# Tavish9/freegaussian

Measured on AMD Instinct MI355X. Metric: Mpixels/s fwd+bwd @ 1M Gaussians 1080p, higher is better.
Workload: dtype f32; 1 GPU; north-star cfg4: 1000000 Gaussians, 1920x1080, SH degree 3, 1 view per rank per step, view = (rank + step) mod 8 around the 8-view ring, fwd+bwd, RGB, absgrad; layout=uniform, N=1000000, P=2073600, parallelism=view-dp1

## Files before the change

freegaussian_amd/csrc/fg_common.h:

```cpp
#pragma once
#include <hip/hip_runtime.h>
#include <stdint.h>

#include "../../include/fgraster.h"

#define FG_WAVE 64

#define FG_RETURN_IF_LAUNCH_FAILED()                  \
  do {                                                \
    if (hipGetLastError() != hipSuccess) return FG_ERR_LAUNCH; \
  } while (0)

static inline hipStream_t fg_hip_stream(fg_stream_t s) { return reinterpret_cast<hipStream_t>(s); }

#define FG_ALPHA_SKIP (1.0f / 255.0f)
#define FG_ALPHA_MAX 0.999f
#define FG_T_STOP 1e-4f
#define FG_FOV_CLAMP 1.3f

namespace fg {

__device__ __forceinline__ int lane_id() { return __lane_id(); }

__device__ __forceinline__ int alpha_extent(float o, float a, float b, float c, float& ex, float& ey) {
// ... 213 lines not shown
  __builtin_amdgcn_wave_barrier();
  __builtin_amdgcn_fence(__ATOMIC_ACQUIRE, "wavefront");
  float r = 0.f;
  if ((lane >> 2) < ROWS) {
    const float4* src = reinterpret_cast<const float4*>(buf + (lane >> 2) * FG_RED_STRIDE + (lane & 3) * 16);
    const float4 a = src[0], b = src[1], c = src[2], d = src[3];
    r = (((a.x + a.y) + (a.z + a.w)) + ((b.x + b.y) + (b.z + b.w))) +
        (((c.x + c.y) + (c.z + c.w)) + ((d.x + d.y) + (d.z + d.w)));
    r += dpp_mov<FG_DPP_QUAD_XOR1>(r);
    r += dpp_mov<FG_DPP_QUAD_XOR2>(r);
  }
  return r;
}

}
```

freegaussian_amd/csrc/preprocess.hip:

```cpp
#include "project_math.h"
#include "sh_math.h"
#include "slab_io.h"

#include <stdlib.h>

namespace {
using namespace fgp;
using namespace fgsh;

constexpr int REC = FG_SPLAT_FLOATS;
constexpr int RSTRIDE = 20;
constexpr int JAC = FG_SH_JAC_FLOATS;
constexpr int JSTRIDE = 11;

struct FeatLayout {
  int sh_degree;
  int k_stored;
  int n_color;
  int with_depth;
  int n_extra;
};

struct RawForm {
  int enabled;
// ... 267 lines not shown
}

template <bool NOTE>
__global__ void __launch_bounds__(BLOCK) __attribute__((amdgpu_waves_per_eu(NOTE ? FG_PRE_BWD_WAVES : 3)))
preprocess_bwd_kernel(int N, FeatLayout fl, RawForm raw, float* __restrict__ v_d_quats,
                      float* __restrict__ v_d_scales, float* __restrict__ v_features_rest,
                      float* __restrict__ v_rgb, int v_rgb_floats,
                      const float* __restrict__ means, const float* __restrict__ quats,
                      const float* __restrict__ scales, const float* __restrict__ opacities,
                      const float* __restrict__ colors, const float* __restrict__ viewmat,
                      const float* __restrict__ K, int width, int height, float eps2d, int antialiased,
                      const int32_t* __restrict__ radii, const float* __restrict__ v_splats,
                      const float* __restrict__ v_means2d, int m2_stride, const float* __restrict__ v_depths,
                      const float* __restrict__ v_conics, float* __restrict__ v_means, float* __restrict__ v_quats,
                      float* __restrict__ v_scales, float* __restrict__ v_opacities, float* __restrict__ v_colors,
                      float* __restrict__ v_extra, const float* __restrict__ sh_jac, int skip_culled) {
  __shared__ float lds[HROWS * ROW];
  __shared__ uint8_t row_live[BLOCK];
  const int row0 = blockIdx.x * BLOCK;
  const int nrows = min(BLOCK, N - row0);
  const int i = row0 + threadIdx.x;
  const int kk = fl.sh_degree >= 0 ? (fl.sh_degree + 1) * (fl.sh_degree + 1) : 0;
  const bool active = (i < N) && radii[i] > 0;
  float sh_dx = 0.f, sh_dy = 0.f, sh_dz = 1.f, sh_inv = 0.f;
  auto view_direction = [&]() { view_dir(viewmat, means[3 * i], means[3 * i + 1], means[3 * i + 2], sh_dx, sh_dy, sh_dz, sh_inv); };
  if (!NOTE && active && kk > 0) view_direction();
  ShSums sums;
#pragma unroll
  for (int c = 0; c < 3; ++c) sums.col[c] = 0.f;
#pragma unroll
  for (int c = 0; c < 9; ++c) sums.jac[c] = 0.f;
// ... 125 lines not shown
    v_scales[3 * i] = g_s[0]; v_scales[3 * i + 1] = g_s[1]; v_scales[3 * i + 2] = g_s[2];
    v_opacities[i] = g_o;
  }
  if (v_rgb && i < N) {
    float* o = v_rgb + (size_t)v_rgb_floats * i;
    o[0] = vr; o[1] = vg; o[2] = vb;
    if (v_rgb_floats == 6) {
      o[3] = sh_dx; o[4] = sh_dy; o[5] = sh_dz;
    }
  }
  if (kk > 0 && v_colors) {
    float basis[16];
#pragma unroll
    for (int k = 0; k < 16; ++k) basis[k] = 0.f;
    if (active) sh_basis(fl.sh_degree, sh_dx, sh_dy, sh_dz, basis);
#pragma unroll
    for (int h = 0; h < 2; ++h) {
      const int r0 = row0 + h * HROWS, nr = min(HROWS, nrows - h * HROWS);
      if (nr <= 0) break;
      __syncthreads();
      if ((int)(threadIdx.x / HROWS) == h) {
        float* row = lds + (threadIdx.x & (HROWS - 1)) * ROW;
#pragma unroll
        for (int k = 0; k < 16; ++k) {
          const float bk = (k < kk) ? basis[k] : 0.f;
          row[3 * k] = bk * vr; row[3 * k + 1] = bk * vg; row[3 * k + 2] = bk * vb;
        }
      }
      __syncthreads();
      if (raw.enabled) {
        lds_to_slab_at<ROW, true, HROWS>(v_colors + (size_t)r0 * 3, lds, 0, nr, 3, 3);
        if (fl.k_stored > 1)
          lds_to_slab_at<ROW, true, HROWS>(v_features_rest + (size_t)r0 * 3 * (fl.k_stored - 1), lds, 3, nr,
                                           3 * (fl.k_stored - 1), 45);
      } else {
        lds_to_slab_at<ROW, true, HROWS>(v_colors + (size_t)r0 * 3 * fl.k_stored, lds, 0, nr, 3 * fl.k_stored, 48);
      }
    }
  }
}

constexpr int VM_BLOCK = 256, VM_GRID_MAX = 1024, VM_VALUES = 15;
__global__ void __launch_bounds__(VM_BLOCK)
viewmat_bwd_kernel(int N, FeatLayout fl, RawForm raw, const float* __restrict__ means, const float* __restrict__ quats,
                   const float* __restrict__ scales, const float* __restrict__ opacities, const float* __restrict__ colors,
                   const float* __restrict__ viewmat, const float* __restrict__ K, int width, int height, float eps2d,
                   int antialiased, const int32_t* __restrict__ radii, const float* __restrict__ v_splats,
                   const float* __restrict__ v_means2d, int m2_stride, const float* __restrict__ v_depths,
                   const float* __restrict__ v_conics, const float* __restrict__ sh_jac, float* __restrict__ partials) {
  __shared__ float red[VM_BLOCK / 64][16];
  float acc[VM_VALUES];
// ... 169 lines not shown
                     depths, conics, compensations, tiles_touched, splats, depth_keys,
                     reinterpret_cast<int2*>(tile_rects), reinterpret_cast<unsigned long long*>(tile_masks), sh_jac,
                     skip_culled_rows());
  FG_RETURN_IF_LAUNCH_FAILED();
  return FG_OK;
}

int launch_preprocess_bwd(int N, RawForm raw, float* v_d_quats, float* v_d_scales, float* v_features_rest,
                          float* v_rgb, int v_rgb_floats,
                          const float* means, const float* quats, const float* scales, const float* opacities,
                          const float* colors, int sh_degree, int k_stored, int n_color, int with_depth, int n_extra,
                          const float* viewmat, const float* K, int width, int height, float eps2d, int antialiased,
                          const int32_t* radii, const float* v_splats, const float* v_means2d, int v_means2d_stride,
                          const float* v_depths, const float* v_conics, float* v_means, float* v_quats,
                          float* v_scales, float* v_opacities, float* v_colors, float* v_extra,
                          const float* sh_jac, fg_stream_t stream) {
  FeatLayout fl{sh_degree, k_stored, sh_degree >= 0 ? 3 : n_color, with_depth ? 1 : 0, n_extra};
  if (N < 0 || width <= 0 || height <= 0 || !layout_ok(fl) || v_means2d_stride < 2) return FG_ERR_INVALID_ARG;
  if (N == 0) return FG_OK;
  if (!means || !quats || !scales || !opacities || !viewmat || !K || !radii || !v_splats || !v_means2d ||
      !v_means || !v_quats || !v_scales || !v_opacities)
    return FG_ERR_INVALID_ARG;
  if ((fl.n_color > 0 && (!colors || (!v_colors && !(v_rgb && sh_degree >= 0)))) || (n_extra > 0 && !v_extra))
    return FG_ERR_INVALID_ARG;
  if (v_rgb && sh_degree < 0) return FG_ERR_UNSUPPORTED;
  if (v_rgb && v_rgb_floats != 3 && v_rgb_floats != 6) return FG_ERR_INVALID_ARG;
  if (raw.enabled) {
    if (sh_degree < 0 || (k_stored > 1 && (!raw.features_rest || (!v_features_rest && !v_rgb)))) return FG_ERR_INVALID_ARG;
    if (v_rgb && (v_colors || v_features_rest)) return FG_ERR_INVALID_ARG;
    if ((raw.d_quats != nullptr) != (v_d_quats != nullptr) || (raw.d_scales != nullptr) != (v_d_scales != nullptr))
      return FG_ERR_INVALID_ARG;
  }
  const bool note = sh_jac != nullptr && sh_degree >= 1;
  hipLaunchKernelGGL(note ? preprocess_bwd_kernel<true> : preprocess_bwd_kernel<false>, dim3((N + BLOCK - 1) / BLOCK),
                     dim3(BLOCK), 0, fg_hip_stream(stream), N, fl, raw, v_d_quats, v_d_scales, v_features_rest, v_rgb, v_rgb_floats, means, quats, scales, opacities, colors,
                     viewmat, K, width, height, eps2d, antialiased, radii, v_splats, v_means2d, v_means2d_stride,
                     v_depths, v_conics, v_means, v_quats, v_scales, v_opacities, v_colors, v_extra, sh_jac,
                     skip_culled_rows());
  FG_RETURN_IF_LAUNCH_FAILED();
  return FG_OK;
}

}

extern "C" int fg_preprocess_fwd(int N, const float* means, const float* quats, const float* scales,
                                 const float* opacities, const float* colors, int sh_degree, int k_stored,
                                 int n_color, int with_depth, const float* extra, int n_extra,
                                 const float* viewmat, const float* K, int width, int height, float eps2d,
                                 float near_plane, float far_plane, float radius_clip, int tile_size,
                                 int antialiased, int32_t* radii, float* means2d, float* depths, float* conics,
                                 float* compensations, int32_t* tiles_touched, float* splats,
                                 uint32_t* depth_keys, int32_t* tile_rects, uint64_t* tile_masks, float* sh_jac,
                                 fg_stream_t stream) {
  return launch_preprocess_fwd(N, RawForm{0, nullptr, nullptr, nullptr}, means, quats, scales, opacities, colors,
                               sh_degree, k_stored, n_color, with_depth, extra, n_extra, viewmat, K, width, height,
                               eps2d, near_plane, far_plane, radius_clip, tile_size, antialiased, radii, means2d,
                               depths, conics, compensations, tiles_touched, splats, depth_keys, tile_rects, tile_masks,
                               sh_jac, stream);
}

extern "C" int fg_preprocess_bwd(int N, const float* means, const float* quats, const float* scales,
                                 const float* opacities, const float* colors, int sh_degree, int k_stored,
                                 int n_color, int with_depth, int n_extra, const float* viewmat, const float* K,
                                 int width, int height, float eps2d, int antialiased, const int32_t* radii,
                                 const float* v_splats, const float* v_means2d, int v_means2d_stride,
                                 const float* v_depths, const float* v_conics, float* v_means, float* v_quats,
                                 float* v_scales, float* v_opacities, float* v_colors, float* v_extra,
                                 const float* sh_jac, fg_stream_t stream) {
  return launch_preprocess_bwd(N, RawForm{0, nullptr, nullptr, nullptr}, nullptr, nullptr, nullptr, nullptr, 3, means, quats,
                               scales, opacities, colors, sh_degree, k_stored, n_color, with_depth, n_extra, viewmat,
                               K, width, height, eps2d, antialiased, radii, v_splats, v_means2d, v_means2d_stride,
                               v_depths, v_conics, v_means, v_quats, v_scales, v_opacities, v_colors, v_extra,
                               sh_jac, stream);
}

extern "C" int fg_preprocess_raw_fwd(int N, const float* means, const float* quats, const float* d_quats,
                                     const float* log_scales, const float* d_scales,
                                     const float* opacity_logits, const float* features_dc,
                                     const float* features_rest, int sh_degree, int k_stored, int with_depth,
                                     const float* extra, int n_extra, const float* viewmat, const float* K,
                                     int width, int height, float eps2d, float near_plane, float far_plane,
                                     float radius_clip, int tile_size, int antialiased, int32_t* radii,
                                     float* means2d, float* depths, float* conics, float* compensations,
                                     int32_t* tiles_touched, float* splats, uint32_t* depth_keys,
                                     int32_t* tile_rects, uint64_t* tile_masks, float* sh_jac, fg_stream_t stream) {
  return launch_preprocess_fwd(N, RawForm{1, d_quats, d_scales, features_rest}, means, quats, log_scales,
                               opacity_logits, features_dc, sh_degree, k_stored, 3, with_depth, extra, n_extra,
                               viewmat, K, width, height, eps2d, near_plane, far_plane, radius_clip, tile_size,
                               antialiased, radii, means2d, depths, conics, compensations, tiles_touched, splats,
                               depth_keys, tile_rects, tile_masks, sh_jac, stream);
}

extern "C" int fg_preprocess_raw_bwd(int N, const float* means, const float* quats, const float* d_quats,
                                     const float* log_scales, const float* d_scales,
                                     const float* opacity_logits, const float* features_dc,
                                     const float* features_rest, int sh_degree, int k_stored, int with_depth,
                                     int n_extra, const float* viewmat, const float* K, int width, int height,
                                     float eps2d, int antialiased, const int32_t* radii, const float* v_splats,
                                     const float* v_means2d, int v_means2d_stride, const float* v_depths,
                                     const float* v_conics, float* v_means, float* v_quats, float* v_d_quats,
                                     float* v_log_scales, float* v_d_scales, float* v_opacity_logits,
                                     float* v_features_dc, float* v_features_rest, float* v_extra,
                                     const float* sh_jac, fg_stream_t stream) {
  return launch_preprocess_bwd(N, RawForm{1, d_quats, d_scales, features_rest}, v_d_quats, v_d_scales,
                               v_features_rest, nullptr, 3, means, quats, log_scales, opacity_logits, features_dc, sh_degree,
                               k_stored, 3, with_depth, n_extra, viewmat, K, width, height, eps2d, antialiased, radii,
                               v_splats, v_means2d, v_means2d_stride, v_depths, v_conics, v_means, v_quats,
                               v_log_scales, v_opacity_logits, v_features_dc, v_extra, sh_jac, stream);
}

extern "C" int fg_preprocess_raw_bwd_factored(
    int N, const float* means, const float* quats, const float* d_quats, const float* log_scales, const float* d_scales,
    const float* opacity_logits, const float* features_dc, const float* features_rest, int sh_degree, int k_stored,
    int with_depth, int n_extra, const float* viewmat, const float* K, int width, int height, float eps2d, int antialiased,
    const int32_t* radii, const float* v_splats, const float* v_means2d, int v_means2d_stride, const float* v_depths,
    const float* v_conics, float* v_means, float* v_quats, float* v_d_quats, float* v_log_scales, float* v_d_scales,
    float* v_opacity_logits, float* v_rgb, int v_rgb_floats, float* v_extra, const float* sh_jac, fg_stream_t stream) {
  if (!v_rgb) return FG_ERR_INVALID_ARG;
  return launch_preprocess_bwd(N, RawForm{1, d_quats, d_scales, features_rest}, v_d_quats, v_d_scales, nullptr, v_rgb,
                               v_rgb_floats, means, quats, log_scales, opacity_logits, features_dc, sh_degree, k_stored, 3,
                               with_depth, n_extra, viewmat, K, width, height, eps2d, antialiased, radii, v_splats,
                               v_means2d, v_means2d_stride, v_depths, v_conics, v_means, v_quats, v_log_scales,
                               v_opacity_logits, nullptr, v_extra, sh_jac, stream);
// ... 76 lines not shown
```

freegaussian_amd/csrc/raster.hip:

```cpp
#include "fg_common.h"

#include <stdlib.h>
#include <string.h>

#include <type_traits>

#include "jobs_build.h"

namespace {
using namespace fgjobs;

constexpr int TILE = 16;

__host__ __device__ constexpr int rec_vec4(int C) { return (6 + C + 3) / 4; }

__device__ __forceinline__ int tile_of_block(int b, int n, int tile_w, int tile_h, int mode) {
  const int xcd = b & 7, k = b >> 3;
  const int only = ((mode >> 8) & 15) - 1, kmod = mode >> 12;
  mode &= 255;
  if (only >= 0 && xcd != only) return -1;
  if (kmod > 1 && k % kmod != 0) return -1;
  if (mode == 0) {
    const int row = (k / tile_w) * 8 + xcd;
    return row < tile_h ? row * tile_w + (k % tile_w) : -1;
// ... 1412 lines not shown
template <int C, int PPT>
__global__ void __launch_bounds__(256 / PPT)
raster_bwd_kernel(int width, int height, int tile_w, int tile_h, int order_mode, const float4* __restrict__ splats,
                  const int32_t* __restrict__ tile_offsets, const int32_t* __restrict__ flatten_ids,
                  const float* __restrict__ alphas, const int32_t* __restrict__ last_ids,
                  const float* __restrict__ v_render, const float* __restrict__ v_alphas,
                  float* __restrict__ v_splats, Composite comp) {
  constexpr int NW = 256 / PPT / 64;
  __shared__ BwdShared<C, 64 * NW> sh;
  const int tile = tile_of_block(blockIdx.x, tile_w * tile_h, tile_w, tile_h, order_mode);
  if (tile < 0) return;
  raster_bwd_body<C, PPT, NW>(sh, tile, 0, width, height, tile_w, splats, tile_offsets, flatten_ids, alphas, last_ids,
                              v_render, v_alphas, v_splats, comp);
}

template <int C, bool LIVE>
__global__ void __launch_bounds__(64)
raster_bwd_mixed_kernel(int width, int height, int tile_w, int tile_h, int nx, int tail_tiles,
                        const int32_t* __restrict__ jobs, int cap,
                        const float4* __restrict__ splats, const int32_t* __restrict__ tile_offsets,
                        const int32_t* __restrict__ flatten_ids, const float* __restrict__ alphas,
                        const int32_t* __restrict__ last_ids, const float* __restrict__ v_render,
                        const float* __restrict__ v_alphas, float* __restrict__ v_splats, Composite comp,
                        Segments seg, const uint32_t* __restrict__ live_words) {
  __shared__ BwdShared<C, 64> sh;
  int strip = -1, part = 0, tile;
  if (seg.parts > 1) {
    if (jobs) {
      tile = share_from_list(blockIdx.x, jobs, cap, part, seg.parts);
    } else {
      const int xcd = blockIdx.x & 7, k = blockIdx.x >> 3;
      const Band band = band_of_xcd(xcd, tile_w, tile_h, nx);
      const int n = band.nrows * band.ncols;
      const int tail = seg.tail > 0 ? min(seg.tail, n) : n, n_main = n - tail;
      int t = k;
      if (k >= n_main) {
        t = n_main + (k - n_main) / seg.parts;
        part = ((k - n_main) - (t - n_main) * seg.parts + t) % seg.parts;
      } else {
        seg.parts = 1;
      }
      tile = job_of_block((t << 3) | xcd, tile_w, tile_h, nx, 0, strip);
    }
  } else {
    tile = jobs ? job_from_list(blockIdx.x, jobs, cap, strip)
                : job_of_block(blockIdx.x, tile_w, tile_h, nx, tail_tiles, strip);
  }
  if (tile < 0) return;
  FG_TL_BEGIN();
  if (seg.prio > 0) {
    const int len = tile_offsets[tile + 1] - tile_offsets[tile];
    job_priority(tile_offsets, tile_w * tile_h, seg.parts > 1 ? len / seg.parts : len, strip < 0 ? 13 : (strip >= 4 ? 10 : 8), seg.prio);
  }
  if (strip < 0)
    raster_bwd_body<C, 4, 1, LIVE>(sh, tile, 0, width, height, tile_w, splats, tile_offsets, flatten_ids, alphas,
                                   last_ids, v_render, v_alphas, v_splats, comp, seg, part, live_words);
  else if (strip >= 4)
    raster_bwd_body<C, 2, 1, LIVE>(sh, tile, strip - 4, width, height, tile_w, splats, tile_offsets, flatten_ids,
                                   alphas, last_ids, v_render, v_alphas, v_splats, comp, seg, part, live_words);
  else
    raster_bwd_body<C, 1, 1, LIVE>(sh, tile, strip, width, height, tile_w, splats, tile_offsets, flatten_ids, alphas,
                                   last_ids, v_render, v_alphas, v_splats, comp, seg, part, live_words);
  FG_TL_END(2, tile, strip, part, seg.parts);
}

__global__ void __launch_bounds__(256)
pack_splats_kernel(int N, int C, const float* __restrict__ means2d, const float* __restrict__ conics,
                   const float* __restrict__ opacities, const float* __restrict__ features,
                   float* __restrict__ splats) {
  const int64_t t = (int64_t)blockIdx.x * blockDim.x + threadIdx.x;
  const int64_t i = t >> 4;
  const int l = (int)(t & 15);
  if (i >= N) return;
  float v = 0.f;
  if (l < 2) v = means2d[2 * i + l];
  else if (l == 2) v = opacities[i];
  else if (l < 6) v = conics[3 * i + (l - 3)];
  else if (l - 6 < C) v = features[(size_t)i * C + (l - 6)];
// ... 296 lines not shown
                         reinterpret_cast<const float4*>(splats), tile_offsets, flatten_ids, render, alphas, last_ids, comp,
                         reinterpret_cast<float4*>(ckpt), live_words, slot_tab);
      hipLaunchKernelGGL(raster_fwd_combine_kernel, dim3(8 * 256), dim3(64), 0, s, width, height, tile_w,
                         local + FG_LOCAL_WORDS, reinterpret_cast<const float4*>(splats), tile_offsets, flatten_ids, render,
                         alphas, last_ids, comp, reinterpret_cast<float4*>(ckpt), live_words, slot_tab);
    }
  }
  return hipGetLastError() == hipSuccess ? FG_OK : FG_ERR_LAUNCH;
}

template <int C>
int launch_bwd_mixed(const Cfg& cfg, int width, int height, int tail, const int32_t* jobs, const float* splats,
                     const int32_t* tile_offsets, const int32_t* flatten_ids, const float* alphas,
                     const int32_t* last_ids, const float* v_render, const float* v_alphas, float* v_splats,
                     Composite comp, hipStream_t s, Segments seg = Segments{nullptr, nullptr, nullptr, 1, 0, 0},
                     const uint32_t* live_words = nullptr) {
  const int tile_w = (width + TILE - 1) / TILE, tile_h = (height + TILE - 1) / TILE;
  const int cap = jobs_cap(cfg, tile_w, tile_h);
  int grid = jobs ? listed_grid(cfg, tile_w, tile_h, tail) : mixed_grid(cfg, tile_w, tile_h, tail);
  if (seg.parts > 1) grid = seg_grid(cfg, tile_w, tile_h, seg.parts, seg.tail, jobs != nullptr);
  if (live_words)
    hipLaunchKernelGGL((raster_bwd_mixed_kernel<C, true>), dim3(grid), dim3(64), 0, s, width, height, tile_w, tile_h, band_nx(cfg), tail,
                       jobs, cap, reinterpret_cast<const float4*>(splats), tile_offsets, flatten_ids, alphas, last_ids,
                       v_render, v_alphas, v_splats, comp, seg, live_words);
  else
    hipLaunchKernelGGL((raster_bwd_mixed_kernel<C, false>), dim3(grid), dim3(64), 0, s, width, height, tile_w, tile_h, band_nx(cfg), tail,
                       jobs, cap, reinterpret_cast<const float4*>(splats), tile_offsets, flatten_ids, alphas, last_ids,
                       v_render, v_alphas, v_splats, comp, seg, live_words);
  return hipGetLastError() == hipSuccess ? FG_OK : FG_ERR_LAUNCH;
}



#define FG_DISPATCH_C(CALL)                  \
  switch (channels) {                        \
    case 1: CALL(1); break;                  \
    case 2: CALL(2); break;                  \
    case 3: CALL(3); break;                  \
    case 4: CALL(4); break;                  \
    case 5: CALL(5); break;                  \
    case 6: CALL(6); break;                  \
    case 7: CALL(7); break;                  \
    case 8: CALL(8); break;                  \
    default: return FG_ERR_UNSUPPORTED;      \
// ... 59 lines not shown
                                      comp, s)                                                                      \
       : (ppt == 2) ? launch_fwd<CC, 2>(cfg, width, height, splats, tile_offsets, flatten_ids, render, alphas, last_ids, \
                                      comp, s)                                                                      \
                    : launch_fwd<CC, 1>(cfg, width, height, splats, tile_offsets, flatten_ids, render, alphas, last_ids, \
                                      comp, s)
  FG_DISPATCH_C(CALL)
#undef CALL
  return rc;
}

int raster_bwd_any(const fg_raster_config* config, int channels, int width, int height, int tile_size, const float* splats,
                   const int32_t* tile_offsets, const int32_t* flatten_ids, const float* alphas,
                   const int32_t* last_ids, const float* v_render, const float* v_alphas, float* v_splats,
                   Composite comp, fg_stream_t stream, const int32_t* jobs = nullptr,
                   const float* seg_ckpt = nullptr, const float* image = nullptr,
                   const uint32_t* live_words = nullptr) {
  if (width <= 0 || height <= 0) return FG_ERR_INVALID_ARG;
  if (tile_size != TILE) return FG_ERR_UNSUPPORTED;
  if (!splats || !tile_offsets || !alphas || !last_ids || !v_render || !v_splats) return FG_ERR_INVALID_ARG;
  if (comp.n_clamp < 0 || comp.n_clamp > channels || (comp.n_clamp > 0 && !comp.clamp_mask)) return FG_ERR_INVALID_ARG;
  hipStream_t s = fg_hip_stream(stream);
  int rc = FG_OK;
  const int n_tiles = ((width + TILE - 1) / TILE) * ((height + TILE - 1) / TILE);
  const Cfg cfg = resolve(config);
  const int ppt = raster_ppt_bwd(cfg, n_tiles);
  int tail = mixed_tail_bwd(cfg, n_tiles);
  if (tail == 0) jobs = nullptr;
  if (mixed_tail_fwd(cfg, n_tiles) == 0) {
    live_words = nullptr;
    seg_ckpt = nullptr;
  }
  Segments seg{nullptr, nullptr, nullptr, 1, 0, 0};
  const int32_t* slot_tab = slot_table(cfg, jobs, (width + TILE - 1) / TILE, (height + TILE - 1) / TILE);
  if (seg_slots(cfg) > 0 && !slot_tab) seg_ckpt = nullptr;
  if (channels == 3 && seg_ckpt && image && tail > 0 && seg_parts(cfg, n_tiles) > 1)
    seg = Segments{reinterpret_cast<float4*>(const_cast<float*>(seg_ckpt)), slot_tab, image, seg_parts(cfg, n_tiles),
                   seg_tail_fit(cfg, (width + TILE - 1) / TILE, (height + TILE - 1) / TILE, seg_parts(cfg, n_tiles),
                                seg_tail(cfg, n_tiles)), 0};
  seg.prio = job_prio(cfg.prio_bwd, FG_PRIO_BWD_DEFAULT);
  seg.fine = seg_fine(cfg);
#define CALL(CC)                                                                                            \
  rc = (tail > 0)   ? launch_bwd_mixed<CC>(cfg, width, height, tail, jobs, splats, tile_offsets, flatten_ids,    \
                                         alphas, last_ids, v_render, v_alphas, v_splats, comp, s, seg,      \
                                         live_use(cfg, live_words))                                              \
       : (ppt == 4) ? launch_bwd<CC, 4>(cfg, width, height, splats, tile_offsets, flatten_ids, alphas, last_ids, \
                                      v_render, v_alphas, v_splats, comp, s)                                \
       : (ppt == 2) ? launch_bwd<CC, 2>(cfg, width, height, splats, tile_offsets, flatten_ids, alphas, last_ids, \
                                      v_render, v_alphas, v_splats, comp, s)                                \
                    : launch_bwd<CC, 1>(cfg, width, height, splats, tile_offsets, flatten_ids, alphas, last_ids, \
                                      v_render, v_alphas, v_splats, comp, s)
  FG_DISPATCH_C(CALL)
#undef CALL
  return rc;
}

}

extern "C" int fg_raster_fwd(int channels, int width, int height, int tile_size, const float* splats,
                             const int32_t* tile_offsets, const int32_t* flatten_ids, float* render,
// ... 123 lines not shown
  return ((int64_t)seg_slots_offset4(n_tiles, width, height) + slots * (int64_t)FG_SEG_SLOT4) * 4;
}

extern "C" int fg_raster_jobs_bwd(int channels, int width, int height, int tile_size, const float* splats,
                                  const int32_t* tile_offsets, const int32_t* flatten_ids, const int32_t* jobs,
                                  const float* background, int n_clamp, const uint8_t* clamp_mask,
                                  const float* alphas, const int32_t* last_ids, const float* v_image,
                                  const float* v_alphas, float* v_splats, const float* seg_ckpt,
                                  const float* image, const uint32_t* live_words, const fg_raster_config* config,
                                  fg_stream_t stream) {
  return raster_bwd_any(config, channels, width, height, tile_size, splats, tile_offsets, flatten_ids, alphas, last_ids,
                        v_image, v_alphas, v_splats, Composite{background, n_clamp, const_cast<uint8_t*>(clamp_mask)},
                        stream, jobs, seg_ckpt, image, live_words);
}

#ifdef FG_RASTER_STATS
extern "C" int fg_debug_raster_stats(unsigned long long* out, int reset) {
  if (hipMemcpyFromSymbol(out, HIP_SYMBOL(fg_raster_stats), sizeof(unsigned long long) * 16) != hipSuccess)
    return FG_ERR_LAUNCH;
  if (reset) {
    unsigned long long z[16] = {0};
    if (hipMemcpyToSymbol(HIP_SYMBOL(fg_raster_stats), z, sizeof(z)) != hipSuccess) return FG_ERR_LAUNCH;
  }
  return FG_OK;
}
#endif

#ifdef FG_RASTER_TIMELINE
extern "C" int fg_debug_raster_timeline(unsigned long long* out, int cap, int reset) {
  unsigned n = 0;
// ... 13 lines not shown
```

freegaussian_amd/csrc/slab_io.h:

```cpp
#pragma once
#include "sh_math.h"

#ifndef FG_SLAB_NT
#define FG_SLAB_NT 1
#endif
#if FG_SLAB_NT
typedef float fg_f4_native __attribute__((ext_vector_type(4)));
__device__ __forceinline__ float4 fg_slab_load_nt(const float4* p) {
  const fg_f4_native v = __builtin_nontemporal_load(reinterpret_cast<const fg_f4_native*>(p));
  return make_float4(v.x, v.y, v.z, v.w);
}
__device__ __forceinline__ void fg_slab_store_nt(float4* p, float4 v) {
  fg_f4_native n = {v.x, v.y, v.z, v.w};
  __builtin_nontemporal_store(n, reinterpret_cast<fg_f4_native*>(p));
}
#define FG_SLAB_LOAD(p) fg_slab_load_nt(p)
#define FG_SLAB_STORE(p, v) fg_slab_store_nt((p), (v))
#else
#define FG_SLAB_LOAD(p) (*(p))
#define FG_SLAB_STORE(p, v) (*(p) = (v))
#endif

namespace fgsh {

// ... 60 lines not shown
          const int cc = wrap ? c + jj - row_floats : c + jj;
          const int row_base = (wrap ? r + 1 : r) * STRIDE;
          lds[row_base + (cc < use_floats ? lds_col0 + cc : STRIDE - 1)] = vv[jj];
        }
      }
    }
  } else {
    const int tot = nrows * use_floats;
    for (int e = threadIdx.x; e < tot; e += BLOCK) {
      const int r = e / use_floats, c = e - r * use_floats;
      if (!row_live || row_live[r]) lds[r * STRIDE + lds_col0 + c] = src[(size_t)r * row_floats + c];
    }
  }
}

template <int STRIDE = ROW, bool NT = true, int MAXROWS = BLOCK>
__device__ __forceinline__ void lds_to_slab_at(float* __restrict__ dst, const float* lds, int lds_col0, int nrows,
                                               int row_floats, int lds_cols) {
  constexpr int SLAB_MAX_Q = slab_max_q(MAXROWS);
  const int total = nrows * row_floats;
  if ((row_floats & 3) == 0 && (lds_cols & 3) == 0 && (reinterpret_cast<uintptr_t>(dst) & 15) == 0) {
    float4* dst4 = reinterpret_cast<float4*>(dst);
    const int rq = row_floats >> 2, lq = lds_cols >> 2, total4 = nrows * rq;
    const unsigned magic = ((1u << 20) + rq - 1) / rq;
#pragma unroll
    for (int t = 0; t < SLAB_MAX_Q; ++t) {
      const int q = threadIdx.x + t * BLOCK;
      if (q < total4) {
        const int r = (int)(((unsigned)q * magic) >> 20), cq = q - r * rq;
        const float* s = lds + r * STRIDE + (cq < lq ? lds_col0 + 4 * cq : 0);
        float4 o = make_float4(s[0], s[1], s[2], s[3]);
        if (cq >= lq) o = make_float4(0.f, 0.f, 0.f, 0.f);
        if (NT) FG_SLAB_STORE(&dst4[q], o);
        else dst4[q] = o;
      }
    }
  } else if ((total & 3) == 0 && (reinterpret_cast<uintptr_t>(dst) & 15) == 0) {
    float4* dst4 = reinterpret_cast<float4*>(dst);
    const int total4 = total / 4;
    const unsigned magic = ((1u << 20) + row_floats - 1) / row_floats;
#pragma unroll
    for (int t = 0; t < SLAB_MAX_Q; ++t) {
      const int q = threadIdx.x + t * BLOCK;
      if (q < total4) {
        const int e = 4 * q;
        const int r = (int)(((unsigned)e * magic) >> 20), c = e - r * row_floats;
        float vv[4];
#pragma unroll
        for (int jj = 0; jj < 4; ++jj) {
          const bool wrap = c + jj >= row_floats;
          const int cc = wrap ? c + jj - row_floats : c + jj;
          const int row_base = (wrap ? r + 1 : r) * STRIDE;
          const float x = lds[row_base + (cc < lds_cols ? lds_col0 + cc : STRIDE - 1)];
          vv[jj] = cc < lds_cols ? x : 0.f;
        }
        if (NT) FG_SLAB_STORE(&dst4[q], make_float4(vv[0], vv[1], vv[2], vv[3]));
        else dst4[q] = make_float4(vv[0], vv[1], vv[2], vv[3]);
      }
    }
  } else {
    for (int e = threadIdx.x; e < total; e += BLOCK) {
      const int r = e / row_floats, c = e - r * row_floats;
      dst[e] = (c < lds_cols) ? lds[r * STRIDE + lds_col0 + c] : 0.f;
    }
  }
}

}
```

freegaussian_amd/csrc/step.hip:

```cpp
#include <string.h>

#include "fg_common.h"

namespace {

size_t al256(size_t x) { return (x + 255) & ~(size_t)255; }

int channels_of(const fg_step_desc& d) {
  const int ncol = d.sh_degree >= 0 ? 3 : d.n_color;
  return ncol + (d.with_depth ? 1 : 0) + d.n_extra;
}

bool desc_ok(const fg_step_desc* d) {
  if (!d || d->size < (int32_t)sizeof(fg_step_desc)) return false;
  if (d->N <= 0 || d->width <= 0 || d->height <= 0 || d->tile_size != 16 || d->capacity <= 0) return false;
  if (d->raw && d->sh_degree < 0) return false;
  const int c = channels_of(*d);
  return c >= 1 && c <= FG_MAX_CHANNELS && d->n_clamp >= 0 && d->n_clamp <= c;
}

template <typename T>
T* at(void* base, const fg_step_layout* L, int which) {
  return L->nbytes[which] > 0 ? reinterpret_cast<T*>(static_cast<char*>(base) + L->offset[which]) : nullptr;
}
// ... 106 lines not shown
  if (io->ev_raster_end && hipEventRecord(static_cast<hipEvent_t>(io->ev_raster_end), fg_hip_stream(stream)) != hipSuccess)
    return FG_ERR_LAUNCH;
  return rc;
}

extern "C" int fg_step_bwd(const fg_step_desc* d, const fg_raster_config* config, const fg_step_io* io, void* keep,
                           const fg_step_layout* L, fg_stream_t stream) {
  if (!desc_ok(d) || !io || !keep || !L || !d->want_backward) return FG_ERR_INVALID_ARG;
  if (!io->v_render || !io->v_means || !io->v_quats || !io->v_scales || !io->v_opacities) return FG_ERR_INVALID_ARG;
  const int N = d->N, W = d->width, H = d->height, C = channels_of(*d);
  float* v_splats = at<float>(keep, L, FG_STEP_V_SPLATS);
  const float* splats = at<float>(keep, L, FG_STEP_SPLATS);
  int32_t* jobs = at<int32_t>(keep, L, FG_STEP_JOBS);
  if (io->ev_raster_begin && hipEventRecord(static_cast<hipEvent_t>(io->ev_raster_begin), fg_hip_stream(stream)) != hipSuccess)
    return FG_ERR_LAUNCH;
  int rc = fg_raster_jobs_bwd(C, W, H, 16, splats, at<int32_t>(keep, L, FG_STEP_LIST_OFFSETS),
                              at<int32_t>(keep, L, FG_STEP_FLATTEN_IDS), jobs + L->jobs_words, io->background, d->n_clamp,
                              at<uint8_t>(keep, L, FG_STEP_CLAMP_MASK), at<float>(keep, L, FG_STEP_ALPHAS),
                              at<int32_t>(keep, L, FG_STEP_LAST_IDS), io->v_render, io->v_alphas, v_splats,
                              at<float>(keep, L, FG_STEP_SEG_CKPT), at<float>(keep, L, FG_STEP_RENDER),
                              at<uint32_t>(keep, L, FG_STEP_LIVE), config, stream);
  if (io->ev_raster_end && hipEventRecord(static_cast<hipEvent_t>(io->ev_raster_end), fg_hip_stream(stream)) != hipSuccess)
    return FG_ERR_LAUNCH;
  if (rc != FG_OK) return rc;
  const int32_t* radii = at<int32_t>(keep, L, FG_STEP_RADII);
  const float* sh_jac = at<float>(keep, L, FG_STEP_SH_JAC);
  if (d->raw) {
    if (io->v_rgb)
      return fg_preprocess_raw_bwd_factored(N, io->means, io->quats, io->d_quats, io->scales, io->d_scales, io->opacities,
                                            io->colors, io->features_rest, d->sh_degree, d->k_stored, d->with_depth, d->n_extra,
                                            io->viewmat, io->K, W, H, d->eps2d, d->antialiased, radii, v_splats, v_splats,
                                            FG_SPLAT_FLOATS, io->v_depths, io->v_conics, io->v_means, io->v_quats, io->v_d_quats,
                                            io->v_scales, io->v_d_scales, io->v_opacities, io->v_rgb, io->v_rgb_floats,
                                            io->v_extra, sh_jac, stream);
    return fg_preprocess_raw_bwd(N, io->means, io->quats, io->d_quats, io->scales, io->d_scales, io->opacities, io->colors,
                                 io->features_rest, d->sh_degree, d->k_stored, d->with_depth, d->n_extra, io->viewmat, io->K, W,
                                 H, d->eps2d, d->antialiased, radii, v_splats, v_splats, FG_SPLAT_FLOATS, io->v_depths,
                                 io->v_conics, io->v_means, io->v_quats, io->v_d_quats, io->v_scales, io->v_d_scales, io->v_opacities,
                                 io->v_colors, io->v_features_rest, io->v_extra, sh_jac, stream);
  }
  if (io->v_rgb)
    return fg_preprocess_bwd_factored(N, io->means, io->quats, io->scales, io->opacities, io->colors, d->sh_degree, d->k_stored,
                                      d->with_depth, d->n_extra, io->viewmat, io->K, W, H, d->eps2d, d->antialiased, radii,
                                      v_splats, v_splats, FG_SPLAT_FLOATS, io->v_depths, io->v_conics, io->v_means, io->v_quats,
                                      io->v_scales, io->v_opacities, io->v_rgb, io->v_rgb_floats, io->v_extra, sh_jac, stream);
  return fg_preprocess_bwd(N, io->means, io->quats, io->scales, io->opacities, io->colors, d->sh_degree, d->k_stored, d->n_color,
                           d->with_depth, d->n_extra, io->viewmat, io->K, W, H, d->eps2d, d->antialiased, radii, v_splats,
                           v_splats, FG_SPLAT_FLOATS, io->v_depths, io->v_conics, io->v_means, io->v_quats, io->v_scales, io->v_opacities,
                           io->v_colors, io->v_extra, sh_jac, stream);
}
```

Measured before the change: 2886 Mpix/s.

## Zero SH gradient rows during raster backward and skip dead rows in preprocess

The raster backward kernel now also zero-fills the SH colour gradient buffer with nontemporal stores, by default after each block finishes its tile. Preprocess backward then writes only the chunks whose rows carry a nonzero colour gradient and skips stores for dead rows. The aim is to overlap the bulk zeroing with the latency-bound raster work and cut the large 48-float-per-Gaussian gradient write traffic in preprocess. The cost is extra store traffic inside the raster kernel and a correctness dependency on the fill having actually run, which is signalled through the prezeroed flag.

```diff
diff --git a/freegaussian_amd/csrc/check/sparse_sh_rows.cpp b/freegaussian_amd/csrc/check/sparse_sh_rows.cpp
--- /dev/null
+++ b/freegaussian_amd/csrc/check/sparse_sh_rows.cpp
@@ -0,0 +1,56 @@
+#include <cstdlib>
+#include <vector>
+
+#include "check_common.h"
+#include "../slab_rows.h"
+
+static std::vector<int> pitches() {
+  std::vector<int> p;
+  for (int k = 1; k <= 16; ++k) p.push_back(3 * k);
+  p.push_back(45);
+  return p;
+}
+
+int main() {
+  unsigned seed = 12345u;
+  auto rnd = [&]() { return (seed = seed * 1664525u + 1013904223u) >> 16; };
+  long long chunks = 0;
+  for (int pitch : pitches())
+    for (int nrows = 1; nrows <= 64; ++nrows) {
+      const int total = nrows * pitch, nq = (total + 3) / 4;
+      for (int q = 0; q < nq; ++q) {
+        int first = -1, last = -1;
+        fgsh::slab_chunk_rows(q, pitch, nrows, first, last);
+        int want_first = nrows, want_last = -1;
+        for (int e = 4 * q; e < 4 * q + 4 && e < total; ++e) {
+          const int r = e / pitch;
+          want_first = r < want_first ? r : want_first;
+          want_last = r > want_last ? r : want_last;
+        }
+        EXPECT(first, want_first);
+        EXPECT(last, want_last);
+        EXPECT(last - first <= 1, 1);
+        ++chunks;
+      }
+      std::vector<unsigned char> live(nrows);
+      for (int r = 0; r < nrows; ++r) live[r] = (rnd() % 4) == 0;
+      std::vector<int> written(4 * nq, 0);
+      for (int q = 0; q < nq; ++q) {
+        int first, last;
+        fgsh::slab_chunk_rows(q, pitch, nrows, first, last);
+        if (live[first] | live[last])
+          for (int e = 4 * q; e < 4 * q + 4; ++e) written[e] = 1;
+      }
+      int missed = 0, needless = 0;
+      for (int e = 0; e < total; ++e) missed += live[e / pitch] && !written[e];
+      for (int q = 0; q < nq; ++q) {
+        bool any = false;
+        for (int e = 4 * q; e < 4 * q + 4 && e < total; ++e) any = any || live[e / pitch];
+        needless += written[4 * q] && !any;
+      }
+      EXPECT(missed, 0);
+      EXPECT(needless, 0);
+    }
+  EXPECT(chunks > 100000, 1);
+  return report("sparse_sh_rows");
+}
diff --git a/freegaussian_amd/csrc/fg_common.h b/freegaussian_amd/csrc/fg_common.h
--- a/freegaussian_amd/csrc/fg_common.h
+++ b/freegaussian_amd/csrc/fg_common.h
@@ -251,3 +251,24 @@
 }
 
 }
+
+__attribute__((visibility("hidden"))) int fg_raster_jobs_bwd_fill(
+    int channels, int width, int height, int tile_size, const float* splats, const int32_t* tile_offsets,
+    const int32_t* flatten_ids, const int32_t* jobs, const float* background, int n_clamp, const uint8_t* clamp_mask,
+    const float* alphas, const int32_t* last_ids, const float* v_image, const float* v_alphas, float* v_splats,
+    const float* seg_ckpt, const float* image, const uint32_t* live_words, float* zero_buf, int64_t zero_floats, int* filled,
+    const fg_raster_config* config, fg_stream_t stream);
+__attribute__((visibility("hidden"))) int fg_preprocess_bwd_prezeroed(
+    int N, const float* means, const float* quats, const float* scales, const float* opacities, const float* colors,
+    int sh_degree, int k_stored, int n_color, int with_depth, int n_extra, const float* viewmat, const float* K, int width,
+    int height, float eps2d, int antialiased, const int32_t* radii, const float* v_splats, const float* v_means2d,
+    int v_means2d_stride, const float* v_depths, const float* v_conics, float* v_means, float* v_quats, float* v_scales,
+    float* v_opacities, float* v_colors, float* v_extra, const float* sh_jac, int rows_prezeroed, fg_stream_t stream);
+__attribute__((visibility("hidden"))) int fg_preprocess_raw_bwd_prezeroed(
+    int N, const float* means, const float* quats, const float* d_quats, const float* log_scales, const float* d_scales,
+    const float* opacity_logits, const float* features_dc, const float* features_rest, int sh_degree, int k_stored,
+    int with_depth, int n_extra, const float* viewmat, const float* K, int width, int height, float eps2d, int antialiased,
+    const int32_t* radii, const float* v_splats, const float* v_means2d, int v_means2d_stride, const float* v_depths,
+    const float* v_conics, float* v_means, float* v_quats, float* v_d_quats, float* v_log_scales, float* v_d_scales,
+    float* v_opacity_logits, float* v_features_dc, float* v_features_rest, float* v_extra, const float* sh_jac,
+    int rows_prezeroed, fg_stream_t stream);
diff --git a/freegaussian_amd/csrc/preprocess.hip b/freegaussian_amd/csrc/preprocess.hip
--- a/freegaussian_amd/csrc/preprocess.hip
+++ b/freegaussian_amd/csrc/preprocess.hip
@@ -305,7 +305,8 @@
                       const float* __restrict__ v_means2d, int m2_stride, const float* __restrict__ v_depths,
                       const float* __restrict__ v_conics, float* __restrict__ v_means, float* __restrict__ v_quats,
                       float* __restrict__ v_scales, float* __restrict__ v_opacities, float* __restrict__ v_colors,
-                      float* __restrict__ v_extra, const float* __restrict__ sh_jac, int skip_culled) {
+                      float* __restrict__ v_extra, const float* __restrict__ sh_jac, int skip_culled,
+                      int rows_prezeroed) {
   __shared__ float lds[HROWS * ROW];
   __shared__ uint8_t row_live[BLOCK];
   const int row0 = blockIdx.x * BLOCK;
@@ -461,6 +462,7 @@
 #pragma unroll
     for (int k = 0; k < 16; ++k) basis[k] = 0.f;
     if (active) sh_basis(fl.sh_degree, sh_dx, sh_dy, sh_dz, basis);
+    if (rows_prezeroed) row_live[threadIdx.x] = !(vr == 0.f && vg == 0.f && vb == 0.f);
 #pragma unroll
     for (int h = 0; h < 2; ++h) {
       const int r0 = row0 + h * HROWS, nr = min(HROWS, nrows - h * HROWS);
@@ -475,13 +477,14 @@
         }
       }
       __syncthreads();
+      const uint8_t* live = rows_prezeroed ? row_live + h * HROWS : nullptr;
       if (raw.enabled) {
         lds_to_slab_at<ROW, true, HROWS>(v_colors + (size_t)r0 * 3, lds, 0, nr, 3, 3);
         if (fl.k_stored > 1)
           lds_to_slab_at<ROW, true, HROWS>(v_features_rest + (size_t)r0 * 3 * (fl.k_stored - 1), lds, 3, nr,
-                                           3 * (fl.k_stored - 1), 45);
+                                           3 * (fl.k_stored - 1), 45, live);
       } else {
-        lds_to_slab_at<ROW, true, HROWS>(v_colors + (size_t)r0 * 3 * fl.k_stored, lds, 0, nr, 3 * fl.k_stored, 48);
+        lds_to_slab_at<ROW, true, HROWS>(v_colors + (size_t)r0 * 3 * fl.k_stored, lds, 0, nr, 3 * fl.k_stored, 48, live);
       }
     }
   }
@@ -681,7 +684,7 @@
                           const int32_t* radii, const float* v_splats, const float* v_means2d, int v_means2d_stride,
                           const float* v_depths, const float* v_conics, float* v_means, float* v_quats,
                           float* v_scales, float* v_opacities, float* v_colors, float* v_extra,
-                          const float* sh_jac, fg_stream_t stream) {
+                          const float* sh_jac, fg_stream_t stream, int rows_prezeroed = 0) {
   FeatLayout fl{sh_degree, k_stored, sh_degree >= 0 ? 3 : n_color, with_depth ? 1 : 0, n_extra};
   if (N < 0 || width <= 0 || height <= 0 || !layout_ok(fl) || v_means2d_stride < 2) return FG_ERR_INVALID_ARG;
   if (N == 0) return FG_OK;
@@ -703,7 +706,7 @@
                      dim3(BLOCK), 0, fg_hip_stream(stream), N, fl, raw, v_d_quats, v_d_scales, v_features_rest, v_rgb, v_rgb_floats, means, quats, scales, opacities, colors,
                      viewmat, K, width, height, eps2d, antialiased, radii, v_splats, v_means2d, v_means2d_stride,
                      v_depths, v_conics, v_means, v_quats, v_scales, v_opacities, v_colors, v_extra, sh_jac,
-                     skip_culled_rows());
+                     skip_culled_rows(), (rows_prezeroed && !v_rgb && sh_degree >= 0) ? 1 : 0);
   FG_RETURN_IF_LAUNCH_FAILED();
   return FG_OK;
 }
@@ -734,11 +737,24 @@
                                  const float* v_depths, const float* v_conics, float* v_means, float* v_quats,
                                  float* v_scales, float* v_opacities, float* v_colors, float* v_extra,
                                  const float* sh_jac, fg_stream_t stream) {
+  return fg_preprocess_bwd_prezeroed(N, means, quats, scales, opacities, colors, sh_degree, k_stored, n_color, with_depth,
+                                     n_extra, viewmat, K, width, height, eps2d, antialiased, radii, v_splats, v_means2d,
+                                     v_means2d_stride, v_depths, v_conics, v_means, v_quats, v_scales, v_opacities, v_colors,
+                                     v_extra, sh_jac, 0, stream);
+}
+
+int fg_preprocess_bwd_prezeroed(int N, const float* means, const float* quats, const float* scales, const float* opacities,
+                                const float* colors, int sh_degree, int k_stored, int n_color, int with_depth, int n_extra,
+                                const float* viewmat, const float* K, int width, int height, float eps2d, int antialiased,
+                                const int32_t* radii, const float* v_splats, const float* v_means2d, int v_means2d_stride,
+                                const float* v_depths, const float* v_conics, float* v_means, float* v_quats, float* v_scales,
+                                float* v_opacities, float* v_colors, float* v_extra, const float* sh_jac, int rows_prezeroed,
+                                fg_stream_t stream) {
   return launch_preprocess_bwd(N, RawForm{0, nullptr, nullptr, nullptr}, nullptr, nullptr, nullptr, nullptr, 3, means, quats,
                                scales, opacities, colors, sh_degree, k_stored, n_color, with_depth, n_extra, viewmat,
                                K, width, height, eps2d, antialiased, radii, v_splats, v_means2d, v_means2d_stride,
                                v_depths, v_conics, v_means, v_quats, v_scales, v_opacities, v_colors, v_extra,
-                               sh_jac, stream);
+                               sh_jac, stream, rows_prezeroed);
 }
 
 extern "C" int fg_preprocess_raw_fwd(int N, const float* means, const float* quats, const float* d_quats,
@@ -769,11 +785,27 @@
                                      float* v_log_scales, float* v_d_scales, float* v_opacity_logits,
                                      float* v_features_dc, float* v_features_rest, float* v_extra,
                                      const float* sh_jac, fg_stream_t stream) {
+  return fg_preprocess_raw_bwd_prezeroed(N, means, quats, d_quats, log_scales, d_scales, opacity_logits, features_dc,
+                                         features_rest, sh_degree, k_stored, with_depth, n_extra, viewmat, K, width, height,
+                                         eps2d, antialiased, radii, v_splats, v_means2d, v_means2d_stride, v_depths, v_conics,
+                                         v_means, v_quats, v_d_quats, v_log_scales, v_d_scales, v_opacity_logits, v_features_dc,
+                                         v_features_rest, v_extra, sh_jac, 0, stream);
+}
+
+int fg_preprocess_raw_bwd_prezeroed(int N, const float* means, const float* quats, const float* d_quats,
+                                    const float* log_scales, const float* d_scales, const float* opacity_logits,
+                                    const float* features_dc, const float* features_rest, int sh_degree, int k_stored,
+                                    int with_depth, int n_extra, const float* viewmat, const float* K, int width, int height,
+                                    float eps2d, int antialiased, const int32_t* radii, const float* v_splats,
+                                    const float* v_means2d, int v_means2d_stride, const float* v_depths, const float* v_conics,
+                                    float* v_means, float* v_quats, float* v_d_quats, float* v_log_scales, float* v_d_scales,
+                                    float* v_opacity_logits, float* v_features_dc, float* v_features_rest, float* v_extra,
+                                    const float* sh_jac, int rows_prezeroed, fg_stream_t stream) {
   return launch_preprocess_bwd(N, RawForm{1, d_quats, d_scales, features_rest}, v_d_quats, v_d_scales,
                                v_features_rest, nullptr, 3, means, quats, log_scales, opacity_logits, features_dc, sh_degree,
                                k_stored, 3, with_depth, n_extra, viewmat, K, width, height, eps2d, antialiased, radii,
                                v_splats, v_means2d, v_means2d_stride, v_depths, v_conics, v_means, v_quats,
-                               v_log_scales, v_opacity_logits, v_features_dc, v_extra, sh_jac, stream);
+                               v_log_scales, v_opacity_logits, v_features_dc, v_extra, sh_jac, stream, rows_prezeroed);
 }
 
 extern "C" int fg_preprocess_raw_bwd_factored(
diff --git a/freegaussian_amd/csrc/raster.hip b/freegaussian_amd/csrc/raster.hip
--- a/freegaussian_amd/csrc/raster.hip
+++ b/freegaussian_amd/csrc/raster.hip
@@ -1450,6 +1450,12 @@
                               v_render, v_alphas, v_splats, comp);
 }
 
+#ifndef FG_BWD_FILL_NT
+#define FG_BWD_FILL_NT 1
+#endif
+#ifndef FG_BWD_FILL_AT_END
+#define FG_BWD_FILL_AT_END 1
+#endif
 template <int C, bool LIVE>
 __global__ void __launch_bounds__(64)
 raster_bwd_mixed_kernel(int width, int height, int tile_w, int tile_h, int nx, int tail_tiles,
@@ -1458,8 +1464,27 @@
                         const int32_t* __restrict__ flatten_ids, const float* __restrict__ alphas,
                         const int32_t* __restrict__ last_ids, const float* __restrict__ v_render,
                         const float* __restrict__ v_alphas, float* __restrict__ v_splats, Composite comp,
-                        Segments seg, const uint32_t* __restrict__ live_words) {
+                        Segments seg, const uint32_t* __restrict__ live_words, float4* __restrict__ zero4,
+                        long long zero_n4) {
   __shared__ BwdShared<C, 64> sh;
+  auto fill = [&]() {
+    if (zero4) {
+      const long long per = (zero_n4 + gridDim.x - 1) / gridDim.x;
+      const long long z0 = per * blockIdx.x, z1 = min(zero_n4, z0 + per);
+      for (long long z = z0 + fg::lane_id(); z < z1; z += 64) {
+#if FG_BWD_FILL_NT
+        typedef float f4n __attribute__((ext_vector_type(4)));
+        const f4n zz = {0.f, 0.f, 0.f, 0.f};
+        __builtin_nontemporal_store(zz, reinterpret_cast<f4n*>(&zero4[z]));
+#else
+        zero4[z] = make_float4(0.f, 0.f, 0.f, 0.f);
+#endif
+      }
+    }
+  };
+#if !FG_BWD_FILL_AT_END
+  fill();
+#endif
   int strip = -1, part = 0, tile;
   if (seg.parts > 1) {
     if (jobs) {
@@ -1482,7 +1507,11 @@
     tile = jobs ? job_from_list(blockIdx.x, jobs, cap, strip)
                 : job_of_block(blockIdx.x, tile_w, tile_h, nx, tail_tiles, strip);
   }
+#if FG_BWD_FILL_AT_END
+  if (tile < 0) { fill(); return; }
+#else
   if (tile < 0) return;
+#endif
   FG_TL_BEGIN();
   if (seg.prio > 0) {
     const int len = tile_offsets[tile + 1] - tile_offsets[tile];
@@ -1498,6 +1527,9 @@
     raster_bwd_body<C, 1, 1, LIVE>(sh, tile, strip, width, height, tile_w, splats, tile_offsets, flatten_ids, alphas,
                                    last_ids, v_render, v_alphas, v_splats, comp, seg, part, live_words);
   FG_TL_END(2, tile, strip, part, seg.parts);
+#if FG_BWD_FILL_AT_END
+  fill();
+#endif
 }
 
 __global__ void __launch_bounds__(256)
@@ -1824,20 +1856,26 @@
                      const int32_t* tile_offsets, const int32_t* flatten_ids, const float* alphas,
                      const int32_t* last_ids, const float* v_render, const float* v_alphas, float* v_splats,
                      Composite comp, hipStream_t s, Segments seg = Segments{nullptr, nullptr, nullptr, 1, 0, 0},
-                     const uint32_t* live_words = nullptr) {
+                     const uint32_t* live_words = nullptr, float* zero_buf = nullptr, long long zero_floats = 0,
+                     int* filled = nullptr) {
   const int tile_w = (width + TILE - 1) / TILE, tile_h = (height + TILE - 1) / TILE;
   const int cap = jobs_cap(cfg, tile_w, tile_h);
   int grid = jobs ? listed_grid(cfg, tile_w, tile_h, tail) : mixed_grid(cfg, tile_w, tile_h, tail);
   if (seg.parts > 1) grid = seg_grid(cfg, tile_w, tile_h, seg.parts, seg.tail, jobs != nullptr);
+  if (zero_floats <= 0 || (zero_floats & 3) || (reinterpret_cast<uintptr_t>(zero_buf) & 15)) zero_buf = nullptr;
+  float4* const zero4 = reinterpret_cast<float4*>(zero_buf);
+  const long long zero_n4 = zero_buf ? zero_floats / 4 : 0ll;
   if (live_words)
     hipLaunchKernelGGL((raster_bwd_mixed_kernel<C, true>), dim3(grid), dim3(64), 0, s, width, height, tile_w, tile_h, band_nx(cfg), tail,
                        jobs, cap, reinterpret_cast<const float4*>(splats), tile_offsets, flatten_ids, alphas, last_ids,
-                       v_render, v_alphas, v_splats, comp, seg, live_words);
+                       v_render, v_alphas, v_splats, comp, seg, live_words, zero4, zero_n4);
   else
     hipLaunchKernelGGL((raster_bwd_mixed_kernel<C, false>), dim3(grid), dim3(64), 0, s, width, height, tile_w, tile_h, band_nx(cfg), tail,
                        jobs, cap, reinterpret_cast<const float4*>(splats), tile_offsets, flatten_ids, alphas, last_ids,
-                       v_render, v_alphas, v_splats, comp, seg, live_words);
-  return hipGetLastError() == hipSuccess ? FG_OK : FG_ERR_LAUNCH;
+                       v_render, v_alphas, v_splats, comp, seg, live_words, zero4, zero_n4);
+  if (hipGetLastError() != hipSuccess) return FG_ERR_LAUNCH;
+  if (filled) *filled = zero_buf != nullptr;
+  return FG_OK;
 }
 
 
@@ -1927,8 +1965,10 @@
                    const int32_t* last_ids, const float* v_render, const float* v_alphas, float* v_splats,
                    Composite comp, fg_stream_t stream, const int32_t* jobs = nullptr,
                    const float* seg_ckpt = nullptr, const float* image = nullptr,
-                   const uint32_t* live_words = nullptr) {
-  if (width <= 0 || height <= 0) return FG_ERR_INVALID_ARG;
+                   const uint32_t* live_words = nullptr, float* zero_buf = nullptr, long long zero_floats = 0,
+                   int* filled = nullptr) {
+  if (filled) *filled = 0;
+  if (width <= 0 || height <= 0 || zero_floats < 0) return FG_ERR_INVALID_ARG;
   if (tile_size != TILE) return FG_ERR_UNSUPPORTED;
   if (!splats || !tile_offsets || !alphas || !last_ids || !v_render || !v_splats) return FG_ERR_INVALID_ARG;
   if (comp.n_clamp < 0 || comp.n_clamp > channels || (comp.n_clamp > 0 && !comp.clamp_mask)) return FG_ERR_INVALID_ARG;
@@ -1955,7 +1995,7 @@
 #define CALL(CC)                                                                                            \
   rc = (tail > 0)   ? launch_bwd_mixed<CC>(cfg, width, height, tail, jobs, splats, tile_offsets, flatten_ids,    \
                                          alphas, last_ids, v_render, v_alphas, v_splats, comp, s, seg,      \
-                                         live_use(cfg, live_words))                                              \
+                                         live_use(cfg, live_words), zero_buf, zero_floats, filled)               \
        : (ppt == 4) ? launch_bwd<CC, 4>(cfg, width, height, splats, tile_offsets, flatten_ids, alphas, last_ids, \
                                       v_render, v_alphas, v_splats, comp, s)                                \
        : (ppt == 2) ? launch_bwd<CC, 2>(cfg, width, height, splats, tile_offsets, flatten_ids, alphas, last_ids, \
@@ -2109,6 +2149,17 @@
                         stream, jobs, seg_ckpt, image, live_words);
 }
 
+int fg_raster_jobs_bwd_fill(int channels, int width, int height, int tile_size, const float* splats,
+                            const int32_t* tile_offsets, const int32_t* flatten_ids, const int32_t* jobs,
+                            const float* background, int n_clamp, const uint8_t* clamp_mask, const float* alphas,
+                            const int32_t* last_ids, const float* v_image, const float* v_alphas, float* v_splats,
+                            const float* seg_ckpt, const float* image, const uint32_t* live_words, float* zero_buf,
+                            int64_t zero_floats, int* filled, const fg_raster_config* config, fg_stream_t stream) {
+  return raster_bwd_any(config, channels, width, height, tile_size, splats, tile_offsets, flatten_ids, alphas, last_ids,
+                        v_image, v_alphas, v_splats, Composite{background, n_clamp, const_cast<uint8_t*>(clamp_mask)},
+                        stream, jobs, seg_ckpt, image, live_words, zero_buf, (long long)zero_floats, filled);
+}
+
 #ifdef FG_RASTER_STATS
 extern "C" int fg_debug_raster_stats(unsigned long long* out, int reset) {
   if (hipMemcpyFromSymbol(out, HIP_SYMBOL(fg_raster_stats), sizeof(unsigned long long) * 16) != hipSuccess)
diff --git a/freegaussian_amd/csrc/slab_io.h b/freegaussian_amd/csrc/slab_io.h
--- a/freegaussian_amd/csrc/slab_io.h
+++ b/freegaussian_amd/csrc/slab_io.h
@@ -1,5 +1,6 @@
 #pragma once
 #include "sh_math.h"
+#include "slab_rows.h"
 
 #ifndef FG_SLAB_NT
 #define FG_SLAB_NT 1
@@ -98,9 +99,16 @@
   }
 }
 
+__device__ __forceinline__ bool chunk_live(const uint8_t* row_live, int q, int row_floats, int nrows) {
+  if (!row_live) return true;
+  int first, last;
+  slab_chunk_rows(q, row_floats, nrows, first, last);
+  return (row_live[first] | row_live[last]) != 0;
+}
+
 template <int STRIDE = ROW, bool NT = true, int MAXROWS = BLOCK>
 __device__ __forceinline__ void lds_to_slab_at(float* __restrict__ dst, const float* lds, int lds_col0, int nrows,
-                                               int row_floats, int lds_cols) {
+                                               int row_floats, int lds_cols, const uint8_t* row_live = nullptr) {
   constexpr int SLAB_MAX_Q = slab_max_q(MAXROWS);
   const int total = nrows * row_floats;
   if ((row_floats & 3) == 0 && (lds_cols & 3) == 0 && (reinterpret_cast<uintptr_t>(dst) & 15) == 0) {
@@ -110,7 +118,7 @@
 #pragma unroll
     for (int t = 0; t < SLAB_MAX_Q; ++t) {
       const int q = threadIdx.x + t * BLOCK;
-      if (q < total4) {
+      if (q < total4 && chunk_live(row_live, q, row_floats, nrows)) {
         const int r = (int)(((unsigned)q * magic) >> 20), cq = q - r * rq;
         const float* s = lds + r * STRIDE + (cq < lq ? lds_col0 + 4 * cq : 0);
         float4 o = make_float4(s[0], s[1], s[2], s[3]);
@@ -126,7 +134,7 @@
 #pragma unroll
     for (int t = 0; t < SLAB_MAX_Q; ++t) {
       const int q = threadIdx.x + t * BLOCK;
-      if (q < total4) {
+      if (q < total4 && chunk_live(row_live, q, row_floats, nrows)) {
         const int e = 4 * q;
         const int r = (int)(((unsigned)e * magic) >> 20), c = e - r * row_floats;
         float vv[4];
@@ -145,7 +153,7 @@
   } else {
     for (int e = threadIdx.x; e < total; e += BLOCK) {
       const int r = e / row_floats, c = e - r * row_floats;
-      dst[e] = (c < lds_cols) ? lds[r * STRIDE + lds_col0 + c] : 0.f;
+      if (!row_live || row_live[r]) dst[e] = (c < lds_cols) ? lds[r * STRIDE + lds_col0 + c] : 0.f;
     }
   }
 }
diff --git a/freegaussian_amd/csrc/slab_rows.h b/freegaussian_amd/csrc/slab_rows.h
--- /dev/null
+++ b/freegaussian_amd/csrc/slab_rows.h
@@ -0,0 +1,19 @@
+#pragma once
+
+#if defined(__HIP__)
+#define FG_SLAB_HD __host__ __device__ inline __attribute__((always_inline))
+#else
+#define FG_SLAB_HD inline
+#endif
+
+namespace fgsh {
+
+FG_SLAB_HD void slab_chunk_rows(int q, int row_floats, int nrows, int& first, int& last) {
+  const unsigned magic = ((1u << 20) + row_floats - 1) / row_floats;
+  const unsigned e = 4u * (unsigned)q;
+  first = (int)((e * magic) >> 20);
+  const int r2 = (int)(((e + 3u) * magic) >> 20);
+  last = r2 < nrows ? r2 : nrows - 1;
+}
+
+}
diff --git a/freegaussian_amd/csrc/step.hip b/freegaussian_amd/csrc/step.hip
--- a/freegaussian_amd/csrc/step.hip
+++ b/freegaussian_amd/csrc/step.hip
@@ -144,12 +144,20 @@
   int32_t* jobs = at<int32_t>(keep, L, FG_STEP_JOBS);
   if (io->ev_raster_begin && hipEventRecord(static_cast<hipEvent_t>(io->ev_raster_begin), fg_hip_stream(stream)) != hipSuccess)
     return FG_ERR_LAUNCH;
-  int rc = fg_raster_jobs_bwd(C, W, H, 16, splats, at<int32_t>(keep, L, FG_STEP_LIST_OFFSETS),
-                              at<int32_t>(keep, L, FG_STEP_FLATTEN_IDS), jobs + L->jobs_words, io->background, d->n_clamp,
-                              at<uint8_t>(keep, L, FG_STEP_CLAMP_MASK), at<float>(keep, L, FG_STEP_ALPHAS),
-                              at<int32_t>(keep, L, FG_STEP_LAST_IDS), io->v_render, io->v_alphas, v_splats,
-                              at<float>(keep, L, FG_STEP_SEG_CKPT), at<float>(keep, L, FG_STEP_RENDER),
-                              at<uint32_t>(keep, L, FG_STEP_LIVE), config, stream);
+  float* rows = nullptr;
+  int64_t row_floats = 0;
+  if (!io->v_rgb && d->sh_degree >= 0) {
+    rows = d->raw ? io->v_features_rest : io->v_colors;
+    row_floats = (int64_t)N * 3 * (d->raw ? d->k_stored - 1 : d->k_stored);
+  }
+  int prezeroed = 0;
+  int rc = fg_raster_jobs_bwd_fill(C, W, H, 16, splats, at<int32_t>(keep, L, FG_STEP_LIST_OFFSETS),
+                                   at<int32_t>(keep, L, FG_STEP_FLATTEN_IDS), jobs + L->jobs_words, io->background, d->n_clamp,
+                                   at<uint8_t>(keep, L, FG_STEP_CLAMP_MASK), at<float>(keep, L, FG_STEP_ALPHAS),
+                                   at<int32_t>(keep, L, FG_STEP_LAST_IDS), io->v_render, io->v_alphas, v_splats,
+                                   at<float>(keep, L, FG_STEP_SEG_CKPT), at<float>(keep, L, FG_STEP_RENDER),
+                                   at<uint32_t>(keep, L, FG_STEP_LIVE), rows, rows ? row_floats : 0, &prezeroed, config,
+                                   stream);
   if (io->ev_raster_end && hipEventRecord(static_cast<hipEvent_t>(io->ev_raster_end), fg_hip_stream(stream)) != hipSuccess)
     return FG_ERR_LAUNCH;
   if (rc != FG_OK) return rc;
@@ -163,19 +171,21 @@
                                             FG_SPLAT_FLOATS, io->v_depths, io->v_conics, io->v_means, io->v_quats, io->v_d_quats,
                                             io->v_scales, io->v_d_scales, io->v_opacities, io->v_rgb, io->v_rgb_floats,
                                             io->v_extra, sh_jac, stream);
-    return fg_preprocess_raw_bwd(N, io->means, io->quats, io->d_quats, io->scales, io->d_scales, io->opacities, io->colors,
-                                 io->features_rest, d->sh_degree, d->k_stored, d->with_depth, d->n_extra, io->viewmat, io->K, W,
-                                 H, d->eps2d, d->antialiased, radii, v_splats, v_splats, FG_SPLAT_FLOATS, io->v_depths,
-                                 io->v_conics, io->v_means, io->v_quats, io->v_d_quats, io->v_scales, io->v_d_scales, io->v_opacities,
-                                 io->v_colors, io->v_features_rest, io->v_extra, sh_jac, stream);
+    return fg_preprocess_raw_bwd_prezeroed(N, io->means, io->quats, io->d_quats, io->scales, io->d_scales, io->opacities,
+                                           io->colors, io->features_rest, d->sh_degree, d->k_stored, d->with_depth, d->n_extra,
+                                           io->viewmat, io->K, W, H, d->eps2d, d->antialiased, radii, v_splats, v_splats,
+                                           FG_SPLAT_FLOATS, io->v_depths, io->v_conics, io->v_means, io->v_quats, io->v_d_quats,
+                                           io->v_scales, io->v_d_scales, io->v_opacities, io->v_colors, io->v_features_rest,
+                                           io->v_extra, sh_jac, prezeroed, stream);
   }
   if (io->v_rgb)
     return fg_preprocess_bwd_factored(N, io->means, io->quats, io->scales, io->opacities, io->colors, d->sh_degree, d->k_stored,
                                       d->with_depth, d->n_extra, io->viewmat, io->K, W, H, d->eps2d, d->antialiased, radii,
                                       v_splats, v_splats, FG_SPLAT_FLOATS, io->v_depths, io->v_conics, io->v_means, io->v_quats,
                                       io->v_scales, io->v_opacities, io->v_rgb, io->v_rgb_floats, io->v_extra, sh_jac, stream);
-  return fg_preprocess_bwd(N, io->means, io->quats, io->scales, io->opacities, io->colors, d->sh_degree, d->k_stored, d->n_color,
-                           d->with_depth, d->n_extra, io->viewmat, io->K, W, H, d->eps2d, d->antialiased, radii, v_splats,
-                           v_splats, FG_SPLAT_FLOATS, io->v_depths, io->v_conics, io->v_means, io->v_quats, io->v_scales, io->v_opacities,
-                           io->v_colors, io->v_extra, sh_jac, stream);
+  return fg_preprocess_bwd_prezeroed(N, io->means, io->quats, io->scales, io->opacities, io->colors, d->sh_degree, d->k_stored,
+                                     d->n_color, d->with_depth, d->n_extra, io->viewmat, io->K, W, H, d->eps2d, d->antialiased,
+                                     radii, v_splats, v_splats, FG_SPLAT_FLOATS, io->v_depths, io->v_conics, io->v_means,
+                                     io->v_quats, io->v_scales, io->v_opacities, io->v_colors, io->v_extra, sh_jac, prezeroed,
+                                     stream);
 }
```

New measurement: 2929 Mpix/s, median of 6. 1.5% higher.
